# SamvitJ/Accel

Hardware: AMD Instinct MI355X
Metric: frames/sec 1024x2048 Accel-18 kf=5 (higher is better)
Workload: dtype f32 (storage, accumulation and results; the launch geometries the tuner picks include the fp32 MFMA, Winograd F(2x2,3x3) and, for most layers, 'fp16x2': each fp32 operand as TWO half terms hi + lo (22-23 significant bits, operands centred in the half range by exact powers of two: weights per channel

## Files before the change

### accel_amd/csrc/conv_b3r.hip

```cpp
#include <hip/hip_runtime.h>
#include <cstdlib>
#include "kernels.h"
#include "conv_common.h"
#include "conv_epilogue.h"

typedef __bf16 bf16x8r __attribute__((ext_vector_type(8)));
typedef _Float16 f16x8r __attribute__((ext_vector_type(8)));

__device__ __forceinline__ void split3_pair_r(float v0, float v1, unsigned& q0, unsigned& q1, unsigned& q2)
{
    const unsigned u0 = __builtin_bit_cast(unsigned, v0), u1 = __builtin_bit_cast(unsigned, v1);
    q0 = __builtin_amdgcn_perm(u1, u0, 0x07060302);
    const float r0 = v0 - __builtin_bit_cast(float, u0 & 0xFFFF0000u), r1 = v1 - __builtin_bit_cast(float, u1 & 0xFFFF0000u);
    const unsigned s0 = __builtin_bit_cast(unsigned, r0), s1 = __builtin_bit_cast(unsigned, r1);
    q1 = __builtin_amdgcn_perm(s1, s0, 0x07060302);
    const float t0 = r0 - __builtin_bit_cast(float, s0 & 0xFFFF0000u), t1 = r1 - __builtin_bit_cast(float, s1 & 0xFFFF0000u);
    q2 = __builtin_amdgcn_perm(__builtin_bit_cast(unsigned, t1), __builtin_bit_cast(unsigned, t0), 0x07060302);
}

template <int BM, int BN, int WGM, int WGN, bool FAST, int ABL = 0, int NPL = 3>
__global__ __launch_bounds__(64 * WGM * WGN, (WGM * WGN == 8 && BM * BN <= 128 * 128 ? 4 : 2)) void conv_b3r_kernel(ConvParams p, size_t wplane, int rowsB)
{
    constexpr int BK = 32, LDK = BK + 8;
    constexpr int NTHR = 64 * WGM * WGN;
    constexpr int CPR = BK / 8, RP = NTHR / CPR;
    constexpr int MI = BM / (WGM * 32), NI = BN / (WGN * 32);
    constexpr int AR = BM / RP;
    static_assert(BM % RP == 0, "tile / thread-count mismatch");
    extern __shared__ __attribute__((aligned(16))) unsigned short smem_r[];
    constexpr int STAGE = NPL * BM * LDK;

    const int tid = threadIdx.x, lane = tid & 63, wave = tid >> 6;
    const int wm = wave / WGN, wn = wave % WGN;
    const int nblk = p.MT * p.NT, bid = blockIdx.x;
    const int q8 = nblk >> 3, r8 = nblk & 7, xcd = bid & 7;
    const int swz = (xcd < r8 ? xcd * (q8 + 1) : r8 * (q8 + 1) + (xcd - r8) * q8) + (bid >> 3);
    const int nt = swz % p.NT, mt = swz / p.NT;
    const int m0 = mt * BM, n0 = nt * BN;

    int ph = p.ph, pw = p.pw;
    const unsigned short* wbase = reinterpret_cast<const unsigned short*>(p.w);
    int py = 0, px = 0;
    if (p.deconv2x) {
        py = blockIdx.y >> 1; px = blockIdx.y & 1;
        ph = 1 - py; pw = 1 - px;
        wbase += (size_t)blockIdx.y * p.w_class_stride;
    }
    const __amdgpu_buffer_rsrc_t xr = make_rsrc(p.x, p.x_bytes);
    const int HoWo = p.Ho * p.Wo;
    RangeScale rs; rs.s = 1.f; rs.inv = 1.f;
    if constexpr (NPL == 2) rs = range_prologue(p.xr);
    const float xs = rs.s;

    const int t4 = tid / CPR;
    const int srow = (t4 & ~7) | ((t4 & 1) << 2) | ((t4 >> 1) & 3), scol = (tid % CPR) * 8;
    int a_iy0[AR], a_ix0[AR];
    unsigned a_base[AR];
#pragma unroll
    for (int i = 0; i < AR; ++i) {
        const int m = m0 + srow + RP * i;
        const bool ok = m < p.M;
        const int mm = ok ? m : 0;
        const int n = mm / HoWo, rem = mm - n * HoWo;
        const int oy = rem / p.Wo, ox = rem - oy * p.Wo;
        a_iy0[i] = ok ? oy * p.sh - ph : -(1 << 28);
        a_ix0[i] = ox * p.sw - pw;
        a_base[i] = (unsigned)(((n * p.H * p.W + a_iy0[i] * p.W + a_ix0[i]) * p.xCs) * 4);
    }
    const int KT_all = p.K_pad / BK;
    const int kt_begin = p.ksplit > 1 ? blockIdx.z * p.kt_per_split : 0;
    const int kt_end = p.ksplit > 1 ? min(KT_all, kt_begin + p.kt_per_split) : KT_all;
    const int nk = kt_end - kt_begin;

    f32x4 ralo[1][AR], rahi[1][AR];
    if constexpr ((ABL & 4) != 0) for (int i = 0; i < AR; ++i) { ralo[0][i] = f32x4{1.f, 2.f, 3.f, (float)lane}; rahi[0][i] = ralo[0][i]; }
    const int4* ktab = p.ktab + (p.deconv2x ? blockIdx.y * (p.K_pad / 4 + 48) : 0);
    int4 tk_next = FAST ? ktab[(kt_begin * BK) / 4] : ktab[(kt_begin * BK + scol) / 4];
    int4 tk2_next = ktab[(kt_begin * BK + scol) / 4 + 1];
    auto load_a = [&](int set, int k0) {
        if constexpr ((ABL & 4) != 0) return;
        if constexpr (FAST) {
            int4 tk = tk_next;
            tk.z += scol * 4;
#pragma unroll
            for (int i = 0; i < AR; ++i) {
                const int iy = a_iy0[i] + tk.x, ix = a_ix0[i] + tk.y;
                const bool ok = (unsigned)iy < (unsigned)p.H && (unsigned)ix < (unsigned)p.W;
                const unsigned off = ok ? a_base[i] + (unsigned)tk.z : OOB;
                ralo[set][i] = buf_load4(xr, off);
                rahi[set][i] = buf_load4(xr, ok ? off + 16u : OOB);
            }
            __builtin_amdgcn_sched_barrier(0);
            tk_next = ktab[(k0 + BK) / 4];
        } else {
            const int4 tk = tk_next, tk2 = tk2_next;
            tk_next = ktab[(k0 + BK + scol) / 4];
            tk2_next = ktab[(k0 + BK + scol) / 4 + 1];
#pragma unroll
            for (int i = 0; i < AR; ++i) {
                const int iy = a_iy0[i] + tk.x, ix = a_ix0[i] + tk.y;
                const bool ok = (unsigned)iy < (unsigned)p.H && (unsigned)ix < (unsigned)p.W;
                const int iy2 = a_iy0[i] + tk2.x, ix2 = a_ix0[i] + tk2.y;
                const bool ok2 = (unsigned)iy2 < (unsigned)p.H && (unsigned)ix2 < (unsigned)p.W;
                ralo[set][i] = buf_load4(xr, ok ? a_base[i] + (unsigned)tk.z : OOB);
                rahi[set][i] = buf_load4(xr, ok2 ? a_base[i] + (unsigned)tk2.z : OOB);
            }
        }
    };
    auto store_a = [&](int stage, int set) {
        if constexpr ((ABL & 8) != 0) return;
        unsigned short* a = smem_r + stage * STAGE;
#pragma unroll
        for (int i = 0; i < AR; ++i) {
            if constexpr (NPL == 1) {
                f16x8r h;
#pragma unroll
                for (int e = 0; e < 4; ++e) { h[e] = (_Float16)ralo[set][i][e]; h[4 + e] = (_Float16)rahi[set][i][e]; }
                *reinterpret_cast<i32x4*>(a + (srow + RP * i) * LDK + scol) = __builtin_bit_cast(i32x4, h);
            } else if constexpr (NPL == 2) {
                f16x8r h, l;
#pragma unroll
                for (int e = 0; e < 8; ++e) {
                    const float v = e < 4 ? ralo[set][i][e] : rahi[set][i][e - 4];
                    h[e] = (_Float16)(v * xs);
                    l[e] = (_Float16)__builtin_fmaf(v, xs, -(float)h[e]);
                }
                *reinterpret_cast<i32x4*>(a + (srow + RP * i) * LDK + scol) = __builtin_bit_cast(i32x4, h);
                *reinterpret_cast<i32x4*>(a + (BM + srow + RP * i) * LDK + scol) = __builtin_bit_cast(i32x4, l);
            } else {
                i32x4 q[3];
                unsigned x0, x1, x2;
                split3_pair_r(ralo[set][i][0], ralo[set][i][1], x0, x1, x2); q[0][0] = (int)x0; q[1][0] = (int)x1; q[2][0] = (int)x2;
                split3_pair_r(ralo[set][i][2], ralo[set][i][3], x0, x1, x2); q[0][1] = (int)x0; q[1][1] = (int)x1; q[2][1] = (int)x2;
                split3_pair_r(rahi[set][i][0], rahi[set][i][1], x0, x1, x2); q[0][2] = (int)x0; q[1][2] = (int)x1; q[2][2] = (int)x2;
                split3_pair_r(rahi[set][i][2], rahi[set][i][3], x0, x1, x2); q[0][3] = (int)x0; q[1][3] = (int)x1; q[2][3] = (int)x2;
#pragma unroll
                for (int pl = 0; pl < 3; ++pl) *reinterpret_cast<i32x4*>(a + (pl * BM + srow + RP * i) * LDK + scol) = q[pl];
            }
        }
    };

    const int frow = lane & 31, half = lane >> 5;
    const __amdgpu_buffer_rsrc_t wall = make_rsrc(wbase, (unsigned)(2 * (NPL - 1) * wplane) + (unsigned)((size_t)rowsB * p.K_pad * 2) + (unsigned)(rowsB * 128));
    unsigned b_voff[NI];
#pragma unroll
    for (int j = 0; j < NI; ++j) b_voff[j] = (unsigned)((n0 + (wn * NI + j) * 32 + frow) * 32 + half * 16);
    const unsigned hstep = (unsigned)rowsB * 32u;
    const unsigned plane_b = (unsigned)(2 * wplane);
    i32x4 fbr[2][NI][NPL];
    if constexpr ((ABL & 2) != 0) for (int b_ = 0; b_ < 2; ++b_) for (int j = 0; j < NI; ++j) for (int pl = 0; pl < NPL; ++pl) fbr[b_][j][pl] = i32x4{lane, 1, 2, 3};
    auto load_b = [&](int hs , int buf) {
        if constexpr ((ABL & 2) != 0) return;
#pragma unroll
        for (int j = 0; j < NI; ++j)
#pragma unroll
            for (int pl = 0; pl < NPL; ++pl)
                fbr[buf][j][pl] = __builtin_amdgcn_raw_buffer_load_b128(wall, b_voff[j], (unsigned)pl * plane_b + (unsigned)hs * hstep, 0);
    };

    f32x16 acc[MI][NI];
#pragma unroll
    for (int i = 0; i < MI; ++i)
#pragma unroll
        for (int j = 0; j < NI; ++j)
#pragma unroll
            for (int e = 0; e < 16; ++e) acc[i][j][e] = 0.f;

    const int fk = half * 8;
    i32x4 fa[1][MI][NPL];
    auto read_fa = [&](int stage, int kb, int set) {
        const unsigned short* a = smem_r + stage * STAGE + (wm * MI * 32 + frow) * LDK + fk + kb * 16;
#pragma unroll
        for (int pl = 0; pl < NPL; ++pl)
#pragma unroll
            for (int i = 0; i < MI; ++i) fa[set][i][pl] = *reinterpret_cast<const i32x4*>(a + (pl * BM + i * 32) * LDK);
    };
    auto mma = [&](int set, int buf) {
#pragma unroll
        for (int i = 0; i < MI; ++i)
#pragma unroll
            for (int j = 0; j < NI; ++j) {
                f32x16 c = acc[i][j];
                if constexpr (NPL == 1) {
                    if constexpr ((ABL & 1) != 0) { asm volatile("" :: "v"(fa[set][i][0]), "v"(fbr[buf][j][0])); continue; }
                    acc[i][j] = __builtin_amdgcn_mfma_f32_32x32x16_f16(__builtin_bit_cast(f16x8r, fa[set][i][0]), __builtin_bit_cast(f16x8r, fbr[buf][j][0]), c, 0, 0, 0);
                } else if constexpr (NPL == 2) {
                    const f16x8r a0 = __builtin_bit_cast(f16x8r, fa[set][i][0]), a1 = __builtin_bit_cast(f16x8r, fa[set][i][1]);
                    const f16x8r b0 = __builtin_bit_cast(f16x8r, fbr[buf][j][0]), b1 = __builtin_bit_cast(f16x8r, fbr[buf][j][1]);
                    if constexpr ((ABL & 1) != 0) { asm volatile("" :: "v"(a0), "v"(a1), "v"(b0), "v"(b1)); continue; }
                    c = __builtin_amdgcn_mfma_f32_32x32x16_f16(a1, b0, c, 0, 0, 0);
                    c = __builtin_amdgcn_mfma_f32_32x32x16_f16(a0, b1, c, 0, 0, 0);
                    acc[i][j] = __builtin_amdgcn_mfma_f32_32x32x16_f16(a0, b0, c, 0, 0, 0);
                } else {
                    const bf16x8r a0 = __builtin_bit_cast(bf16x8r, fa[set][i][0]), a1 = __builtin_bit_cast(bf16x8r, fa[set][i][1]),
                                  a2 = __builtin_bit_cast(bf16x8r, fa[set][i][2]);
                    const bf16x8r b0 = __builtin_bit_cast(bf16x8r, fbr[buf][j][0]), b1 = __builtin_bit_cast(bf16x8r, fbr[buf][j][1]),
                                  b2 = __builtin_bit_cast(bf16x8r, fbr[buf][j][2]);
                    if constexpr ((ABL & 1) != 0) {
                        asm volatile("" :: "v"(a0), "v"(a1), "v"(a2), "v"(b0), "v"(b1), "v"(b2));
                        continue;
                    }
                    c = __builtin_amdgcn_mfma_f32_32x32x16_bf16(a1, b1, c, 0, 0, 0);
                    c = __builtin_amdgcn_mfma_f32_32x32x16_bf16(a0, b2, c, 0, 0, 0);
                    c = __builtin_amdgcn_mfma_f32_32x32x16_bf16(a2, b0, c, 0, 0, 0);
                    c = __builtin_amdgcn_mfma_f32_32x32x16_bf16(a0, b1, c, 0, 0, 0);
                    c = __builtin_amdgcn_mfma_f32_32x32x16_bf16(a1, b0, c, 0, 0, 0);
                    acc[i][j] = __builtin_amdgcn_mfma_f32_32x32x16_bf16(a0, b0, c, 0, 0, 0);
                }
            }
    };

    load_a(0, kt_begin * BK);
    load_b(2 * kt_begin, 0);
    store_a(0, 0);
    __syncthreads();
    load_a(0, (kt_begin + 1) * BK);
    constexpr int FENCES = ((BM == 128 && BN == 128 && WGM == 2 && WGN == 4) || WGN == 8) ? 7
                           : (BN == 256 && WGM == 2) ? 1
                           : (BN == 128 && WGM == 1) ? 4 : 0;
#define B3R_FENCE_N(n) do { if constexpr ((FENCES & (n)) != 0) __builtin_amdgcn_sched_barrier(0); } while (0)
    for (int k = 0; k < nk; ++k) {
        const int cur = k & 1, ks = kt_begin + k;
        load_b(2 * ks + 1, 1);
        B3R_FENCE_N(1);
        read_fa(cur, 0, 0);
        mma(0, 0);
        store_a(cur ^ 1, 0);
        B3R_FENCE_N(2);
        load_a(0, (ks + 2) * BK);
        load_b(2 * ks + 2, 0);
        B3R_FENCE_N(4);
        read_fa(cur, 1, 0);
        mma(0, 1);
        if constexpr ((ABL & 16) == 0) __syncthreads();
    }
#undef B3R_FENCE_N
    if constexpr ((ABL & 32) != 0) {
        f32x16 t = acc[0][0];
#pragma unroll
        for (int i = 0; i < MI; ++i)
#pragma unroll
            for (int j = 0; j < NI; ++j) t += acc[i][j];
        if (p.slope == 12345.f)
            for (int e = 0; e < 16; ++e) p.y[threadIdx.x * 16 + e] = t[e];
        return;
    }
    conv_epilogue<MI, NI, WGN>(p, acc, m0, n0, wm, wn, lane, py, px, HoWo, rs.inv);
}

template <int BM, int BN, int WGM, int WGN, int ABL = 0, int NPL = 3>
static hipError_t launch_b3r(const ConvParams& p0, hipStream_t st)
{
    ConvParams p = p0;
    p.MT = (p.M + BM - 1) / BM;
    p.NT = (p.Cout_store + BN - 1) / BN;
    constexpr size_t lds = (size_t)2 * NPL * BM * 40 * sizeof(unsigned short);
    if (hipError_t e = ensure_dynamic_lds(reinterpret_cast<const void*>(&conv_b3r_kernel<BM, BN, WGM, WGN, true, ABL, NPL>), lds); e != hipSuccess) return e;
    if (hipError_t e = ensure_dynamic_lds(reinterpret_cast<const void*>(&conv_b3r_kernel<BM, BN, WGM, WGN, false, ABL, NPL>), lds); e != hipSuccess) return e;
    const int rowsB = (int)(p.w_bytes / ((unsigned)p.K_pad * 2u));
    dim3 grid(p.MT * p.NT, p.deconv2x ? 4 : 1, p.ksplit > 1 ? p.ksplit : 1);
    if (p.Cin % 32 == 0) hipLaunchKernelGGL((conv_b3r_kernel<BM, BN, WGM, WGN, true, ABL, NPL>), grid, dim3(64 * WGM * WGN), lds, st, p, p.w_plane, rowsB);
    else hipLaunchKernelGGL((conv_b3r_kernel<BM, BN, WGM, WGN, false, ABL, NPL>), grid, dim3(64 * WGM * WGN), lds, st, p, p.w_plane, rowsB);
    hipError_t e = hipGetLastError();
    if (e != hipSuccess || p.ksplit <= 1) return e;
    return launch_splitk_reduce(p, (int)grid.y, st);
}

hipError_t launch_conv_b3r(const ConvParams& p, int tile, hipStream_t st)
{
    if (p.f16 == 1) {
        switch (tile) {
            case CONV_TILE_B3R: return launch_b3r<128, 128, 2, 4, 0, 1>(p, st);
            case CONV_TILE_B3R + 1: return launch_b3r<128, 64, 2, 2, 0, 1>(p, st);
            case CONV_TILE_B3R + 3: return launch_b3r<128, 256, 2, 4, 0, 1>(p, st);
            case CONV_TILE_B3R + 4: return launch_b3r<128, 256, 1, 8, 0, 1>(p, st);
            case CONV_TILE_B3R + 5: return launch_b3r<128, 128, 1, 4, 0, 1>(p, st);
            default: return hipErrorInvalidValue;
        }
    }
    if (p.f16 == 3) {
        switch (tile) {
            case CONV_TILE_B3R: return launch_b3r<128, 128, 2, 4, 0, 2>(p, st);
            case CONV_TILE_B3R + 1: return launch_b3r<128, 64, 2, 2, 0, 2>(p, st);
            case CONV_TILE_B3R + 3: return launch_b3r<128, 256, 2, 4, 0, 2>(p, st);
            case CONV_TILE_B3R + 4: return launch_b3r<128, 256, 1, 8, 0, 2>(p, st);
            case CONV_TILE_B3R + 5: return launch_b3r<128, 128, 1, 4, 0, 2>(p, st);
#ifdef ACCEL_CONV_DIAG
            case 90: return launch_b3r<128, 128, 2, 4, 1, 2>(p, st);
            case 91: return launch_b3r<128, 128, 2, 4, 2, 2>(p, st);
            case 92: return launch_b3r<128, 128, 2, 4, 4, 2>(p, st);
            case 93: return launch_b3r<128, 128, 2, 4, 8, 2>(p, st);
            case 94: return launch_b3r<128, 128, 2, 4, 32, 2>(p, st);
            case 95: return launch_b3r<128, 128, 2, 4, 33, 2>(p, st);
            case 96: return launch_b3r<128, 128, 2, 4, 46, 2>(p, st);
#endif
            default: return hipErrorInvalidValue;
        }
    }
    switch (tile) {
        case CONV_TILE_B3R: return launch_b3r<128, 128, 2, 4>(p, st);
        case CONV_TILE_B3R + 1: return launch_b3r<128, 64, 2, 2>(p, st);
        case CONV_TILE_B3R + 3: return launch_b3r<128, 256, 2, 4>(p, st);
        case CONV_TILE_B3R + 4: return launch_b3r<128, 256, 1, 8>(p, st);
        case CONV_TILE_B3R + 5: return launch_b3r<128, 128, 1, 4>(p, st);
#ifdef ACCEL_CONV_DIAG
        case 90: return launch_b3r<128, 128, 2, 4, 1>(p, st);
        case 91: return launch_b3r<128, 128, 2, 4, 2>(p, st);
        case 92: return launch_b3r<128, 128, 2, 4, 4>(p, st);
        case 93: return launch_b3r<128, 128, 2, 4, 8>(p, st);
        case 94: return launch_b3r<128, 128, 2, 4, 16>(p, st);
        case 95: return launch_b3r<128, 128, 2, 4, 14>(p, st);
        case 96: return launch_b3r<128, 128, 2, 4, 30>(p, st);
#endif
        default: return hipErrorInvalidValue;
    }
}
```

Before: 634.7.

## Stage b3r weights in LDS via buffer-to-LDS DMA for 128x256 fp16x2 tile

For the NPL=2, 128x256, 2x4-wave configuration, weight tiles are no longer loaded from global memory into registers by every wave. Each wave instead DMAs one 32-row chunk straight into a triple-buffered LDS ring using buffer_load ... lds, and waves read their B fragments from LDS. The ktab pointer is also marked constant address space so its loads can go through scalar loads. This aims to cut redundant global weight traffic and register pressure, at the cost of more LDS per block (possibly lowering occupancy) and hand-managed vmcnt waits.

```diff
diff --git a/accel_amd/csrc/conv_b3r.hip b/accel_amd/csrc/conv_b3r.hip
--- a/accel_amd/csrc/conv_b3r.hip
+++ b/accel_amd/csrc/conv_b3r.hip
@@ -1,5 +1,6 @@
 #include <hip/hip_runtime.h>
 #include <cstdlib>
+#include <type_traits>
 #include "kernels.h"
 #include "conv_common.h"
 #include "conv_epilogue.h"
@@ -17,6 +18,42 @@
     const float t0 = r0 - __builtin_bit_cast(float, s0 & 0xFFFF0000u), t1 = r1 - __builtin_bit_cast(float, s1 & 0xFFFF0000u);
     q2 = __builtin_amdgcn_perm(__builtin_bit_cast(unsigned, t1), __builtin_bit_cast(unsigned, t0), 0x07060302);
 }
+
+template <int BM, int BN, int WGM, int WGN, int ABL, int NPL>
+constexpr bool b3r_lds_weights()
+{
+#ifdef ACCEL_B3R_GLOBAL_B
+    return false;
+#else
+    return NPL == 2 && ABL == 0 && BM == 128 && BN == 256 && WGM == 2 && WGN == 4;
+#endif
+}
+template <int BM, int BN, int WGM, int WGN, int ABL, int NPL>
+constexpr size_t b3r_lds_bytes()
+{
+    return (size_t)2 * NPL * BM * 40 * sizeof(unsigned short) + (b3r_lds_weights<BM, BN, WGM, WGN, ABL, NPL>() ? (size_t)3 * 2 * NPL * BN * 32 : 0);
+}
+
+__device__ __forceinline__ void b3r_dma_step(i32x4 desc, unsigned voff0, unsigned voff1, unsigned soff0, unsigned soff1,
+                                             unsigned lds00, unsigned lds01, unsigned lds10, unsigned lds11)
+{
+#if defined(__HIP_DEVICE_COMPILE__)
+    unsigned keep;
+    asm volatile("s_mov_b32 %0, m0\n\t"
+                 "s_mov_b32 m0, %6\n\ts_nop 0\n\tbuffer_load_dwordx4 %1, %3, %4 offen lds\n\t"
+                 "s_mov_b32 m0, %7\n\ts_nop 0\n\tbuffer_load_dwordx4 %2, %3, %4 offen lds\n\t"
+                 "s_mov_b32 m0, %8\n\ts_nop 0\n\tbuffer_load_dwordx4 %1, %3, %5 offen lds\n\t"
+                 "s_mov_b32 m0, %9\n\ts_nop 0\n\tbuffer_load_dwordx4 %2, %3, %5 offen lds\n\t"
+                 "s_mov_b32 m0, %0"
+                 : "=&s"(keep)
+                 : "v"(voff0), "v"(voff1), "s"(desc), "s"(soff0), "s"(soff1), "s"(lds00), "s"(lds01), "s"(lds10), "s"(lds11));
+#endif
+}
+#if defined(__HIP_DEVICE_COMPILE__)
+#define B3R_WAIT_VMCNT(n) asm volatile("s_waitcnt vmcnt(%0)" :: "i"(n))
+#else
+#define B3R_WAIT_VMCNT(n) ((void)0)
+#endif
 
 template <int BM, int BN, int WGM, int WGN, bool FAST, int ABL = 0, int NPL = 3>
 __global__ __launch_bounds__(64 * WGM * WGN, (WGM * WGN == 8 && BM * BN <= 128 * 128 ? 4 : 2)) void conv_b3r_kernel(ConvParams p, size_t wplane, int rowsB)
@@ -74,7 +111,15 @@
 
     f32x4 ralo[1][AR], rahi[1][AR];
     if constexpr ((ABL & 4) != 0) for (int i = 0; i < AR; ++i) { ralo[0][i] = f32x4{1.f, 2.f, 3.f, (float)lane}; rahi[0][i] = ralo[0][i]; }
-    const int4* ktab = p.ktab + (p.deconv2x ? blockIdx.y * (p.K_pad / 4 + 48) : 0);
+    const int4* ktab_g = p.ktab + (p.deconv2x ? blockIdx.y * (p.K_pad / 4 + 48) : 0);
+    typedef const int4* ktab_plain_ptr;
+#if defined(__HIP_DEVICE_COMPILE__)
+    typedef const __attribute__((address_space(4))) int4* ktab_const_ptr;
+#else
+    typedef ktab_plain_ptr ktab_const_ptr;
+#endif
+    constexpr bool LDSB_ = b3r_lds_weights<BM, BN, WGM, WGN, ABL, NPL>();
+    const auto ktab = (std::conditional_t<LDSB_, ktab_const_ptr, ktab_plain_ptr>)ktab_g;
     int4 tk_next = FAST ? ktab[(kt_begin * BK) / 4] : ktab[(kt_begin * BK + scol) / 4];
     int4 tk2_next = ktab[(kt_begin * BK + scol) / 4 + 1];
     auto load_a = [&](int set, int k0) {
@@ -147,7 +192,30 @@
     for (int j = 0; j < NI; ++j) b_voff[j] = (unsigned)((n0 + (wn * NI + j) * 32 + frow) * 32 + half * 16);
     const unsigned hstep = (unsigned)rowsB * 32u;
     const unsigned plane_b = (unsigned)(2 * wplane);
-    i32x4 fbr[2][NI][NPL];
+    constexpr bool LDSB = b3r_lds_weights<BM, BN, WGM, WGN, ABL, NPL>();
+    constexpr unsigned WPLANE_B = BN * 32, WHALF_B = NPL * WPLANE_B, WSTEP_B = 2 * WHALF_B;
+    static_assert(!LDSB || (BN / 32 == WGM * WGN && NPL == 2), "one 32-row chunk per wavefront, two planes");
+    const unsigned wlds = (unsigned)(__UINTPTR_TYPE__)(__attribute__((address_space(3))) unsigned short*)smem_r + 2u * STAGE * 2u;
+    const unsigned wave_u = (unsigned)__builtin_amdgcn_readfirstlane(wave);
+    const unsigned long long wb64 = (unsigned long long)wbase;
+    const i32x4 wdesc = {(int)(unsigned)wb64, (int)(unsigned)(wb64 >> 32),
+                         (int)((unsigned)(2 * (NPL - 1) * wplane) + (unsigned)((size_t)rowsB * p.K_pad * 2) + (unsigned)(rowsB * 128)), ACCEL_BUF_FLAGS};
+    const int dma_row = n0 + (int)wave_u * 32 + frow;
+    const unsigned dma_voff0 = dma_row < rowsB ? (unsigned)(dma_row * 32 + half * 16) : OOB;
+    const unsigned dma_voff1 = dma_row < rowsB ? (unsigned)(dma_row * 32 + half * 16) + plane_b : OOB;
+    auto dma_b = [&](int ks , unsigned stage_b ) {
+        const unsigned l = wlds + stage_b + wave_u * 1024u;
+        b3r_dma_step(wdesc, dma_voff0, dma_voff1, (unsigned)(2 * ks) * hstep, (unsigned)(2 * ks + 1) * hstep,
+                     l, l + WPLANE_B, l + WHALF_B, l + WHALF_B + WPLANE_B);
+    };
+    i32x4 fbr[LDSB ? 1 : 2][NI][NPL];
+    auto read_fb = [&](unsigned stage_b, int kb) {
+        const char* b = reinterpret_cast<const char*>(smem_r) + 2 * STAGE * 2 + stage_b + kb * WHALF_B + (wn * NI) * 1024 + lane * 16;
+#pragma unroll
+        for (int pl = 0; pl < NPL; ++pl)
+#pragma unroll
+            for (int j = 0; j < NI; ++j) fbr[0][j][pl] = *reinterpret_cast<const i32x4*>(b + pl * WPLANE_B + j * 1024);
+    };
     if constexpr ((ABL & 2) != 0) for (int b_ = 0; b_ < 2; ++b_) for (int j = 0; j < NI; ++j) for (int pl = 0; pl < NPL; ++pl) fbr[b_][j][pl] = i32x4{lane, 1, 2, 3};
     auto load_b = [&](int hs , int buf) {
         if constexpr ((ABL & 2) != 0) return;
@@ -210,6 +278,39 @@
             }
     };
 
+    if constexpr (LDSB) {
+        [[maybe_unused]] constexpr int DMAS = 2 * NPL;
+        unsigned st_cur = 0, st_nxt = WSTEP_B, st_fil = 2 * WSTEP_B;
+        load_a(0, kt_begin * BK);
+        __builtin_amdgcn_sched_barrier(0);
+        dma_b(kt_begin, st_cur);
+        dma_b(kt_begin + 1, st_nxt);
+        store_a(0, 0);
+        B3R_WAIT_VMCNT(DMAS);
+        __syncthreads();
+        load_a(0, (kt_begin + 1) * BK);
+        for (int k = 0; k < nk; ++k) {
+            const int cur = k & 1, ks = kt_begin + k;
+            __builtin_amdgcn_sched_barrier(0);
+            read_fa(cur, 0, 0);
+            read_fb(st_cur, 0);
+            mma(0, 0);
+            __builtin_amdgcn_sched_barrier(0);
+            store_a(cur ^ 1, 0);
+            __builtin_amdgcn_sched_barrier(0);
+            dma_b(ks + 2, st_fil);
+            load_a(0, (ks + 2) * BK);
+            __builtin_amdgcn_sched_barrier(0);
+            read_fa(cur, 1, 0);
+            read_fb(st_cur, 1);
+            mma(0, 0);
+            __builtin_amdgcn_sched_barrier(0);
+            B3R_WAIT_VMCNT(DMAS + 2 * AR);
+            __syncthreads();
+            const unsigned t = st_cur; st_cur = st_nxt; st_nxt = st_fil; st_fil = t;
+        }
+        B3R_WAIT_VMCNT(0);
+    } else {
     load_a(0, kt_begin * BK);
     load_b(2 * kt_begin, 0);
     store_a(0, 0);
@@ -235,6 +336,7 @@
         if constexpr ((ABL & 16) == 0) __syncthreads();
     }
 #undef B3R_FENCE_N
+    }
     if constexpr ((ABL & 32) != 0) {
         f32x16 t = acc[0][0];
 #pragma unroll
@@ -254,7 +356,8 @@
     ConvParams p = p0;
     p.MT = (p.M + BM - 1) / BM;
     p.NT = (p.Cout_store + BN - 1) / BN;
-    constexpr size_t lds = (size_t)2 * NPL * BM * 40 * sizeof(unsigned short);
+    constexpr size_t lds = b3r_lds_bytes<BM, BN, WGM, WGN, ABL, NPL>();
+    static_assert(lds <= 160 * 1024, "a block's LDS");
     if (hipError_t e = ensure_dynamic_lds(reinterpret_cast<const void*>(&conv_b3r_kernel<BM, BN, WGM, WGN, true, ABL, NPL>), lds); e != hipSuccess) return e;
     if (hipError_t e = ensure_dynamic_lds(reinterpret_cast<const void*>(&conv_b3r_kernel<BM, BN, WGM, WGN, false, ABL, NPL>), lds); e != hipSuccess) return e;
     const int rowsB = (int)(p.w_bytes / ((unsigned)p.K_pad * 2u));
@@ -266,6 +369,23 @@
     return launch_splitk_reduce(p, (int)grid.y, st);
 }
 
+#ifdef ACCEL_CONV_DIAG
+#ifndef ACCEL_DIAG_B3R_BASE
+#define ACCEL_DIAG_B3R_BASE 76
+#endif
+#if ACCEL_DIAG_B3R_BASE == 76
+#define B3R_DIAG_BASE 128, 128, 2, 4
+#elif ACCEL_DIAG_B3R_BASE == 79
+#define B3R_DIAG_BASE 128, 256, 2, 4
+#elif ACCEL_DIAG_B3R_BASE == 80
+#define B3R_DIAG_BASE 128, 256, 1, 8
+#elif ACCEL_DIAG_B3R_BASE == 81
+#define B3R_DIAG_BASE 128, 128, 1, 4
+#else
+#error "ACCEL_DIAG_B3R_BASE: 76, 79, 80 or 81"
+#endif
+#endif
+
 hipError_t launch_conv_b3r(const ConvParams& p, int tile, hipStream_t st)
 {
     if (p.f16 == 1) {
@@ -286,13 +406,13 @@
             case CONV_TILE_B3R + 4: return launch_b3r<128, 256, 1, 8, 0, 2>(p, st);
             case CONV_TILE_B3R + 5: return launch_b3r<128, 128, 1, 4, 0, 2>(p, st);
 #ifdef ACCEL_CONV_DIAG
-            case 90: return launch_b3r<128, 128, 2, 4, 1, 2>(p, st);
-            case 91: return launch_b3r<128, 128, 2, 4, 2, 2>(p, st);
-            case 92: return launch_b3r<128, 128, 2, 4, 4, 2>(p, st);
-            case 93: return launch_b3r<128, 128, 2, 4, 8, 2>(p, st);
-            case 94: return launch_b3r<128, 128, 2, 4, 32, 2>(p, st);
-            case 95: return launch_b3r<128, 128, 2, 4, 33, 2>(p, st);
-            case 96: return launch_b3r<128, 128, 2, 4, 46, 2>(p, st);
+            case 90: return launch_b3r<B3R_DIAG_BASE, 1, 2>(p, st);
+            case 91: return launch_b3r<B3R_DIAG_BASE, 2, 2>(p, st);
+            case 92: return launch_b3r<B3R_DIAG_BASE, 4, 2>(p, st);
+            case 93: return launch_b3r<B3R_DIAG_BASE, 8, 2>(p, st);
+            case 94: return launch_b3r<B3R_DIAG_BASE, 32, 2>(p, st);
+            case 95: return launch_b3r<B3R_DIAG_BASE, 33, 2>(p, st);
+            case 96: return launch_b3r<B3R_DIAG_BASE, 46, 2>(p, st);
 #endif
             default: return hipErrorInvalidValue;
         }
@@ -304,13 +424,13 @@
         case CONV_TILE_B3R + 4: return launch_b3r<128, 256, 1, 8>(p, st);
         case CONV_TILE_B3R + 5: return launch_b3r<128, 128, 1, 4>(p, st);
 #ifdef ACCEL_CONV_DIAG
-        case 90: return launch_b3r<128, 128, 2, 4, 1>(p, st);
-        case 91: return launch_b3r<128, 128, 2, 4, 2>(p, st);
-        case 92: return launch_b3r<128, 128, 2, 4, 4>(p, st);
-        case 93: return launch_b3r<128, 128, 2, 4, 8>(p, st);
-        case 94: return launch_b3r<128, 128, 2, 4, 16>(p, st);
-        case 95: return launch_b3r<128, 128, 2, 4, 14>(p, st);
-        case 96: return launch_b3r<128, 128, 2, 4, 30>(p, st);
+        case 90: return launch_b3r<B3R_DIAG_BASE, 1>(p, st);
+        case 91: return launch_b3r<B3R_DIAG_BASE, 2>(p, st);
+        case 92: return launch_b3r<B3R_DIAG_BASE, 4>(p, st);
+        case 93: return launch_b3r<B3R_DIAG_BASE, 8>(p, st);
+        case 94: return launch_b3r<B3R_DIAG_BASE, 16>(p, st);
+        case 95: return launch_b3r<B3R_DIAG_BASE, 14>(p, st);
+        case 96: return launch_b3r<B3R_DIAG_BASE, 30>(p, st);
 #endif
         default: return hipErrorInvalidValue;
     }
```

Result: slower. 625.0 (-1.5%).
